# exosports/transit

Hardware: AMD Instinct MI355X
Metric: wavenumber-points*layers/sec (CH4 2-4um emission spectrum) (higher is better)
Workload: dtype f64; 1 GPU; BASELINE configs[1]: CH4-demo-shaped emission: 2500-5000 cm-1 @1 cm-1, wnosamp 2160, CH4 lines, eclipse, 5 angles, H2-H2 CIA; n_wn=2501, n_layers=100, layers_needed=81, n_lines=1000000, parallelism=one GPU

## Files before the change

transit_amd/csrc/hip/trx_api.hip:

```cpp
#include <hip/hip_runtime.h>
#include <rccl/rccl.h>
#include <dlfcn.h>

#include <algorithm>
#include <chrono>
#include <cmath>
#include <cstdio>
#include <cstdlib>
#include <cstring>
#include <atomic>
#include <condition_variable>
#include <memory>
#include <mutex>
#include <string>
#include <thread>
#include <vector>

#include "transit_hip.h"
#include "trx_kernels.hip.h"
#include "trx_walk.hip.h"
#include "trx_rows.hip.h"
#include "trx_tail.hip.h"
#include "trx_lanes.hip.h"
#include "trx_bands.hip.h"
// ... 15 lines not shown
  void release() { if (p) { (void)hipFree(p); p = nullptr; bytes = 0; } }
  template <class T> T *as() const { return (T *)p; }
};

struct PinnedBuf {
  void *p = nullptr, *dev = nullptr; size_t bytes = 0;
  ~PinnedBuf() { release(); }
  void release() { if (p) { (void)hipHostFree(p); p = dev = nullptr; bytes = 0; } }
};

struct DevView {
  void *p = nullptr;
  template <class T> T *as() const { return (T *)p; }
};

struct BandSet {
  int32_t nbands = 0; int64_t npieces = 0;
  DevBuf d_bands, d_pieces, d_w, d_part;
  PinnedBuf h_out;
};

struct PixelSet {
  int64_t npix = 0; double cut = 0;
  DevBuf d_centre, d_fwhm;
};
struct ObservedSet {
  int32_t nexp = 0, nseg = 0; int64_t npix = 0;
  DevBuf d_seg, d_data, d_weight, d_gain;
  std::vector<int64_t> seg;
};
struct FilterSet {
  int32_t ncomp = 0, npad = 0, nexp = 0, nseg = 0; int64_t npix = 0, ntiles = 0;
  DevBuf d_fwd, d_back, d_tiles;
};
struct PixelRun { const PixelSet *set; int32_t nshift; const ObservedSet *obs = nullptr; const FilterSet *filt = nullptr; };

struct Switches {
  bool no_row_copy = false;
  bool no_rows32 = false;
  bool row_staging = true;
  long long row_m8_from = 768;
  bool packed_walk = true; int packed_max_layers = 10;
  int xcd_map = 1;
  bool no_binrec = false;
  bool lanes_walk = true, lanes_force = false;
  int lanes_parts_most = 4;
  bool ray_tail = true;
  bool cia_sums = true;
  bool cia_segments = true;
  bool cia_window = true;
  bool two_queues = true;
  bool tail_direct = true;
  bool range_reach = true;
  bool shard_frames = true;
};

}

struct trx_handle {
  int device = 0;
  hipStream_t stream = nullptr, stream2 = nullptr;
  hipStream_t stream4 = nullptr;
  std::vector<hipEvent_t> ev_ac, ev_cb;
  hipEvent_t ev_walk1 = nullptr;
  hipEvent_t ev_inputs = nullptr, ev_cia = nullptr, ev_join = nullptr, ev_run_a = nullptr, ev_run_b = nullptr;
  std::string err;

  double wn_i = 0, wn_d = 0, odwn = 0; int64_t nwn = 0, nown = 0, lo = 0, hi = 0, nsh = 0; int osamp = 1;
  int niso = 0, nmol = 0;
  std::vector<double> iso_mass, iso_ratio, mol_mass, mol_radius, mol_pol;
  std::vector<double> pair_csd, pair_sqrt;
  std::vector<int32_t> iso_imol, mol_is_h2;
  std::vector<double> iso_wmin, iso_wmax;
  int ndop = 0, nlor = 0;
  std::vector<double> adop, alor;
  std::vector<int32_t> psizeT; bool psize_mono = false;
  std::vector<double> dopthr;
  std::vector<double> lorthr;
  std::vector<int> guess_dop, guess_lor, guess_a0, guess_a1;
  std::vector<long> guess_npre;
  std::vector<double> iso_sqrtm;
  std::vector<double> dens_over_m;
  std::vector<int32_t> psize; std::vector<long long> poff; int64_t tab_n = 0;
  DevBuf d_adop, d_dopthr, d_e2tab, d_psize, d_poff, d_tab, d_tabT, d_poffT, d_gimod, d_gidiv;
  float *tab = nullptr; const float *tabT = nullptr; const long long *poffT = nullptr;
  DevBuf d_tabW, d_walkprof; const float *tabW = nullptr; bool tabw_ok = false;
  DevBuf d_tabW32, d_wp32; const float *tabW32 = nullptr; unsigned slab32 = 0;
  std::vector<std::pair<double, double>> recip_ok;
  int max_gcount = 0; DevBuf d_linebase, d_rinfo;
  Switches sw;
  int64_t nlines = 0, ngroups = 0, nadd = 0, ninrange = 0;
  DevBuf d_lgroup, d_wavn, d_elow, d_gf, d_iso, d_inr, d_gfirst, d_gcount, d_giown, d_giso, d_gwavn, d_gblock, d_cntge, d_cntsub;
  int sub_f = 1;
  LinesDev L{};
  HostBuf<double> h_gwavn; std::vector<int32_t> h_gblock; HostBuf<int32_t> h_cntge, h_gfirst, h_gcount;
  void *comm = nullptr; int nranks = 1, rank = 0;
  bool windowed() const { return lo > 0 || hi < nwn; }
  DevBuf d_cand, d_candrec; int64_t ncand = -1;
  DevBuf d_kmax;
  int kmax_parity = 0, kmax_nr = 0; bool kmax_clean = false;
  DevBuf d_walk, d_wbase, d_part[2];
  std::vector<int32_t> h_wbase; int nwaves = 0, ngw = 0; bool walk_ok = false;
  bool walk_temp_ok = true;
  struct Plan { bool built = false; DevBuf blo, bhi, off, binw, binrec; int64_t records = 0; };
  Plan plan[4];
  struct Cia { int nspec; int mol[2]; std::vector<double> wn, temp, cs, zt, uw, ruw, rh, wf, wb; DevBuf d_wn, d_temp, d_cs, d_zt, d_uw, d_ruw, d_rh, d_wf, d_wb; };
  std::vector<Cia> cia;
  DevBuf d_cia_ws;
  DevBuf d_SG, d_idop8, d_sticky, d_part3;
  DevBuf d_in; PinnedBuf h_in;
  DevBuf d_pm_f64, d_pm_i32;
  DevBuf d_xf;
  DevBuf d_small; DevView d_flags, d_status, d_counters; PinnedBuf h_small;
  DevBuf d_e, d_ecs, d_er, d_tau, d_last, d_intens, d_spec, d_acc, d_geom;
  bool has_grid = false; long og_nmol = 0, og_ntemp = 0, og_nlayer = 0, og_nwave = 0;
  std::vector<double> og_temp; std::vector<int32_t> og_molidx; DevBuf d_og_o, d_og_layer, d_og_itemp, d_iso_mx, d_pm;
  trx_stats stats{};
  std::vector<double> run_f64, run_geom, run_ipv; std::vector<int32_t> run_i32;
  std::vector<int> run_frame; std::vector<unsigned char> run_wide;
  std::vector<PlanStep> run_plan;
  std::vector<double> run_og_layer; std::vector<int> run_og_itemp;
  int hint_layers = 0;
  DevBuf d_e_saved; std::vector<uint8_t> saved;
  PinnedBuf h_spec;
  PinnedBuf h_tailblk;
  std::unique_ptr<BandSet> bands;
  DevBuf d_cpart; PinnedBuf h_contrib;
  std::unique_ptr<PixelSet> pixels;
  DevBuf d_pixshift, d_pixout;
  std::unique_ptr<ObservedSet> observed;
  DevBuf d_mom;
  std::unique_ptr<FilterSet> filter;
  DevBuf d_pixval;
};

namespace {

struct LogSink { trx_log_fn fn = nullptr; void *user = nullptr; int max_level = 0; };
LogSink &log_sink() { static LogSink s; return s; }
void log_msg(int level, const std::string &msg)
{
  const LogSink s = log_sink();
// ... 44 lines not shown
int ensure_small(trx_handle *h, int nlay)
{
  const size_t bytes = 128 + 24 * (size_t)nlay;
  if (const int rc = ensure(h, h->d_small, bytes)) return rc;
  char *base = (char *)h->d_small.p;
  h->d_flags.p = base; h->d_status.p = base + 64; h->d_counters.p = base + 128;
  return ensure_pinned(h, h->h_small, bytes);
}

template <class T>
int upload_raw(trx_handle *h, DevBuf &b, const T *p, size_t n)
{
  int rc = ensure(h, b, n * sizeof(T));
  if (rc) return rc;
  if (n) HIPCHK(h, hipMemcpyAsync(b.p, p, n * sizeof(T), hipMemcpyHostToDevice, h->stream));
  return TRX_OK;
}

template <class T>
int upload(trx_handle *h, DevBuf &b, const std::vector<T> &v)
{
  int rc = ensure(h, b, v.size() * sizeof(T));
  if (rc) return rc;
  if (!v.empty()) HIPCHK(h, hipMemcpyAsync(b.p, v.data(), v.size() * sizeof(T), hipMemcpyHostToDevice, h->stream));
  return TRX_OK;
}

template <class T>
int upload(trx_handle *h, DevBuf &b, const HostBuf<T> &v) { return upload_raw(h, b, v.data(), v.size()); }

void read_switches(Switches &w)
{
  auto set = [](const char *name) { return std::getenv(name) != nullptr; };
  auto num = [](const char *name, long long otherwise) { const char *e = std::getenv(name); return e ? std::atoll(e) : otherwise; };
  auto clamped = [&](const char *name, int lo, int hi, int otherwise) { return (int)std::max<long long>(lo, std::min<long long>(hi, num(name, otherwise))); };
  w.no_row_copy = set("TRX_NO_ROW_COPY");
  w.no_rows32 = set("TRX_NO_ROWS32");
  w.row_staging = !set("TRX_NO_ROW_STAGING");
  w.row_m8_from = num("TRX_ROWS_M8_FROM", w.row_m8_from);
  w.packed_walk = !set("TRX_NO_PACKED_WALK");
  w.packed_max_layers = clamped("TRX_PACKED_MAX_LAYERS", 1, 32, w.packed_max_layers);
  w.xcd_map = (int)num("TRX_XCD_MAP", w.xcd_map);
  w.no_binrec = set("TRX_NO_BINREC");
  const long long lanes = num("TRX_LANES_WALK", 1);
  w.lanes_walk = lanes != 0; w.lanes_force = lanes == 2;
  w.lanes_parts_most = clamped("TRX_LANES_PARTS", 2, 4, w.lanes_parts_most);
  w.ray_tail = num("TRX_RAY_TAIL", 1) != 0;
  w.cia_sums = num("TRX_CIA_SUMS", 1) != 0;
  w.cia_segments = num("TRX_CIA_SEGMENTS", 1) != 0;
  w.cia_window = num("TRX_CIA_WINDOW", 1) != 0;
  w.two_queues = num("TRX_TWO_QUEUES", 1) != 0;
  w.tail_direct = num("TRX_TAIL_DIRECT", 1) != 0;
  w.range_reach = num("TRX_RANGE_REACH", 1) != 0;
  w.shard_frames = num("TRX_SHARD_FRAMES", 1) != 0;
}

struct TableBuild { TablePlan P; DevBuf d_jobs; };

template <class F>
void for_job_batches(const std::vector<ProfileJob> &jobs, F fn)
{
  for (size_t j0 = 0; j0 < jobs.size(); j0 += 32768) fn(j0, (int)std::min<size_t>(32768, jobs.size() - j0));
}

int plan_into_handle(trx_handle *h, const trx_static *s, TableBuild &B)
{
  const char *text = "";
  const TablePlanError pe = plan_table(*s, B.P, &text);
  if (pe != kTablePlanOk) return fail(h, pe == kTablePlanArg ? TRX_E_ARG : TRX_E_UNSUPPORTED, text);
  h->adop = B.P.adop; h->alor = B.P.alor; h->psize = B.P.psize; h->poff = B.P.poff; h->tab_n = B.P.tab_n;
  h->psizeT = std::move(B.P.psizeT); h->psize_mono = B.P.psize_mono;
  if (!index_steps(h->adop.data(), s->ndop, h->dopthr)) return fail(h, TRX_E_ARG, "Doppler-width grid is not strictly increasing");
  if (!index_steps(h->alor.data(), s->nlor, h->lorthr)) h->lorthr.clear();
  return TRX_OK;
}

int upload_table_inputs(trx_handle *h, const trx_static *s, TableBuild &B)
{
  int rc;
  double coef[64]; long double fact = 1.0L;
  for (int n = 0; n < 64; n++) { if (n > 0) fact *= (long double)n; coef[n] = (double)(1.0L / (fact * (long double)(2 * n + 1))); }
  HIPCHK(h, hipMemcpyToSymbolAsync(HIP_SYMBOL(c_voigt_coef), coef, sizeof(coef), 0, hipMemcpyHostToDevice, h->stream));
  if ((rc = upload(h, B.d_jobs, B.P.jobs))) return rc;
  const size_t tab_alloc = table_alloc_floats(h->tab_n, s->osamp);
  if ((rc = ensure(h, h->d_tab, sizeof(float) * tab_alloc))) return rc;
  HIPCHK(h, hipMemsetAsync(h->d_tab.p, 0, sizeof(float) * tab_alloc, h->stream));
  h->tab = h->d_tab.as<float>() + kTabPad;
  if ((rc = upload(h, h->d_psize, h->psize)) || (rc = upload(h, h->d_poff, h->poff)) || (rc = upload(h, h->d_adop, h->adop)) ||
      (rc = upload(h, h->d_dopthr, h->dopthr))) return rc;
  std::vector<double> e2(64);
  for (int j = 0; j < 64; j++) e2[j] = (double)exp2l((long double)j / 64.0L);
  return upload(h, h->d_e2tab, e2);
}

void table_kernels(trx_handle *h, const TableBuild &B)
{
  const int m_limit = 64;
  const std::vector<ProfileJob> &jobs = B.P.jobs;
  for_job_batches(jobs, [&](size_t j0, int nj) {
    int maxnv = 0; bool any_wave = false;
    for (int j = 0; j < nj; j++) { maxnv = std::max(maxnv, jobs[j0 + j].nv); any_wave |= (jobs[j0 + j].regime == 2 && jobs[j0 + j].m > m_limit); }
    const int gx = std::max(1, std::min(64, (maxnv + 255) / 256));
    hipLaunchKernelGGL(k_voigt_bins, dim3(gx, nj), dim3(256), 0, h->stream, B.d_jobs.as<ProfileJob>() + j0, h->tab, m_limit);
    if (any_wave)
      hipLaunchKernelGGL(k_voigt_bins_wave, dim3(std::max(1, std::min(256, maxnv)), nj), dim3(64), 0, h->stream,
                         B.d_jobs.as<ProfileJob>() + j0, h->tab, m_limit);
// ... 176 lines not shown
    for (int64_t g = g0; g < g1; g++) { Q.lgroup[(size_t)G.first[g]] = (int32_t)g; Q.gimod[g] = G.iown[g] % s->osamp; Q.gidiv[g] = G.iown[g] / s->osamp; }
  });
  Q.T.lap("cnt_sub, lgroup, gimod");
}

int walk_ranges(trx_handle *h, const trx_static *s, const LinePrep &Q)
{
  h->walk_ok = s->osamp < (1 << 21) && h->tab_n < ((int64_t)1 << 28) && !Q.LG.first.empty();
  if (!h->walk_ok) return TRX_OK;
  const int ngw = h->ngw = groups_per_range((int64_t)Q.LG.first.size());
  h->h_wbase.assign(s->niso + 1, 0);
  for (int b = 0; b < s->niso; b++) h->h_wbase[b + 1] = h->h_wbase[b] + (Q.gblock[b + 1] - Q.gblock[b] + ngw - 1) / ngw;
  h->nwaves = h->h_wbase[s->niso];
  return upload(h, h->d_wbase, h->h_wbase);
}

int upload_lines(trx_handle *h, LinePrep &Q)
{
  LineGroups &G = Q.LG;
  int rc;
  if ((rc = upload(h, h->d_wavn, Q.wavn)) || (rc = upload(h, h->d_inr, Q.inr)) || (rc = upload(h, h->d_lgroup, Q.lgroup)) ||
      (rc = upload(h, h->d_gfirst, G.first)) || (rc = upload(h, h->d_gcount, G.count)) || (rc = upload(h, h->d_giown, G.iown)) ||
      (rc = upload(h, h->d_giso, G.iso)) || (rc = upload(h, h->d_gwavn, G.wavn)) || (rc = upload(h, h->d_gimod, Q.gimod)) ||
      (rc = upload(h, h->d_gidiv, Q.gidiv)) || (rc = upload(h, h->d_gblock, Q.gblock)) || (rc = upload(h, h->d_cntge, Q.cntge)) ||
      (rc = upload(h, h->d_cntsub, Q.cntsub)))
    return rc;
  HIPCHK(h, hipStreamSynchronize(h->stream));
  Q.T.lap("uploads + sync");
  h->h_gwavn = std::move(G.wavn); h->h_gblock = Q.gblock; h->h_cntge = std::move(Q.cntge); h->h_gfirst = std::move(G.first); h->h_gcount = std::move(G.count);
  Q.T.lap("host copies");
  LinesDev &L = h->L;
  L.nlines = Q.n; L.wavn = h->d_wavn.as<double>(); L.elow = h->d_elow.as<double>(); L.gf = h->d_gf.as<double>();
  L.iso = h->d_iso.as<int16_t>(); L.inrange = h->d_inr.as<uint8_t>(); L.lgroup = h->d_lgroup.as<int32_t>();
  L.ngroups = h->ngroups; L.gfirst = h->d_gfirst.as<int32_t>(); L.gcount = h->d_gcount.as<int32_t>();
  L.giown = h->d_giown.as<int32_t>(); L.giso = h->d_giso.as<int16_t>(); L.gwavn = h->d_gwavn.as<double>();
  L.gblock = h->d_gblock.as<int32_t>(); L.cnt_ge = h->d_cntge.as<int32_t>();
  return TRX_OK;
}

int walk_records(trx_handle *h, const trx_static *s, const LinePrep &Q)
{
  const int64_t n = Q.n; const LinesDev &L = h->L;
  int rc;
  if ((rc = ensure(h, h->d_walk, sizeof(WalkLine) * ((size_t)n + 1))) || (rc = ensure(h, h->d_linebase, sizeof(double) * ((size_t)n + 1)))) return rc;
  HIPCHK(h, hipMemsetAsync(h->d_linebase.p, 0, sizeof(double) * ((size_t)n + 1), h->stream));
  h->max_gcount = parallel_minmax<int>((int64_t)h->h_gcount.size(), Q.nth, 0, 0, [&](int64_t g, bool &) { return (int)h->h_gcount[(size_t)g]; }).hi;
  hipLaunchKernelGGL(k_walk_records, dim3((unsigned)((n + 256) / 256)), dim3(256), 0, h->stream, (long long)n, L.wavn, L.elow, L.gf,
                     L.lgroup, L.giown, s->osamp, h->d_walk.as<WalkLine>());
  hipLaunchKernelGGL(k_walk_marks, dim3((unsigned)((h->nwaves + 63) / 64)), dim3(64), 0, h->stream, h->nwaves, h->ngw, s->niso,
                     h->d_wbase.as<int32_t>(), L.gblock, L.gfirst, L.gcount, h->d_walk.as<WalkLine>(), h->d_linebase.as<double>());
  if ((rc = ensure(h, h->d_rinfo, sizeof(RangeInfo) * (size_t)std::max(h->nwaves, 1)))) return rc;
  hipLaunchKernelGGL(k_range_info, dim3((unsigned)((h->nwaves + 255) / 256)), dim3(256), 0, h->stream, h->nwaves, h->ngw, s->niso,
                     h->d_wbase.as<int32_t>(), L.gblock, L.gfirst, L.gcount, h->d_walk.as<WalkLine>(), s->osamp, h->d_rinfo.as<RangeInfo>());
  return TRX_OK;
}

int line_candidates(trx_handle *h, const trx_static *s, const LinePrep &Q)
{
  const int64_t n = Q.n; const LinesDev &L = h->L;
  h->ncand = -1;
  if (!(h->ninrange > 4096 && s->niso > 0)) return TRX_OK;
  const MinMax<double> e = parallel_minmax<double>(n, Q.nth, HUGE_VAL, -HUGE_VAL, [&](int64_t i, bool &use) { use = Q.inr[i]; return s->elow[i]; });
  CandGeom Gm{};
  Gm.e_min = e.lo; Gm.e_scale = e.hi > e.lo ? kCandGrid / (e.hi - e.lo) : 0.0;
  Gm.w_min = Q.wn0;  Gm.w_scale = Q.own_last > Q.wn0 ? kCandGrid / (Q.own_last - Q.wn0) : 0.0;
  const int cap = (int)std::max<int64_t>(4096, n / 8);
  DevBuf d_M, d_n;
  const size_t mbytes = sizeof(unsigned long long) * (size_t)s->niso * kCandGrid * kCandGrid;
  int rc;
  if ((rc = ensure(h, d_M, mbytes)) || (rc = ensure(h, d_n, sizeof(int))) || (rc = ensure(h, h->d_cand, sizeof(int32_t) * (size_t)cap))) return rc;
  HIPCHK(h, hipMemsetAsync(d_M.p, 0, mbytes, h->stream));
  HIPCHK(h, hipMemsetAsync(d_n.p, 0, sizeof(int), h->stream));
  const unsigned nb = (unsigned)((n + 255) / 256);
  hipLaunchKernelGGL(k_cand_cellmax, dim3(nb), dim3(256), 0, h->stream, (long long)n, L.wavn, L.elow, L.gf, L.iso, L.inrange, Gm, d_M.as<unsigned long long>());
  hipLaunchKernelGGL(k_cand_prefix, dim3((unsigned)s->niso), dim3(kCandGrid), 0, h->stream, d_M.as<unsigned long long>());
  hipLaunchKernelGGL(k_cand_select, dim3(nb), dim3(256), 0, h->stream, (long long)n, L.wavn, L.elow, L.gf, L.iso, L.inrange, Gm,
                     d_M.as<unsigned long long>(), h->d_cand.as<int32_t>(), d_n.as<int>(), cap);
  int nc = 0;
  HIPCHK(h, hipMemcpyAsync(&nc, d_n.p, sizeof(int), hipMemcpyDeviceToHost, h->stream));
  HIPCHK(h, hipStreamSynchronize(h->stream));
  HIPCHK(h, hipGetLastError());
  if (!(nc > 0 && nc <= cap)) return TRX_OK;
  h->ncand = nc;
  if ((rc = ensure(h, h->d_candrec, sizeof(CandLine) * (size_t)nc))) return rc;
  hipLaunchKernelGGL(k_cand_pack, dim3((unsigned)((nc + 255) / 256)), dim3(256), 0, h->stream, nc, h->d_cand.as<int32_t>(),
                     L.wavn, L.elow, L.gf, L.iso, L.inrange, h->d_candrec.as<CandLine>());
  HIPCHK(h, hipStreamSynchronize(h->stream));
  return TRX_OK;
}

int prepare_lines(trx_handle *h, const trx_static *s)
{
  LinePrep Q;
  const int64_t n = Q.n = s->nlines;
  Q.nth = create_threads();
  Q.wn0 = s->wn_i; Q.odwn = s->wn_d / s->osamp; Q.own_last = Q.wn0 + (double)(s->nown - 1) * Q.odwn;
  if (n > 2000000000LL) return fail(h, TRX_E_UNSUPPORTED, "more than 2^31 lines per handle");
  int rc_raw = TRX_OK;
  std::thread raw_up([&]() {
    (void)hipSetDevice(h->device);
    if ((rc_raw = upload_raw(h, h->d_elow, s->elow, (size_t)n)) || (rc_raw = upload_raw(h, h->d_gf, s->gf, (size_t)n)) ||
        (rc_raw = upload_raw(h, h->d_iso, s->isoid, (size_t)n))) return;
  });
  struct Joiner { std::thread &t; ~Joiner() { if (t.joinable()) t.join(); } } raw_join{raw_up};
  int rc;
  if ((rc = line_wavenumbers(h, s, Q)) || (rc = check_line_order(h, s, Q)) || (rc = group_and_check(h, s, Q))) return rc;
// ... 435 lines not shown

template <int NB>
void launch_walk(const WalkArgs &A, bool prof, unsigned nwaves, hipStream_t st)
{
  const dim3 grid((nwaves + kWalkWaves - 1) / kWalkWaves), block(64 * kWalkWaves);
  if (prof) hipLaunchKernelGGL((k_line_walk<NB, true>), grid, block, 0, st, A);
  else if constexpr (NB >= 8) {
    if (A.nc <= 32) hipLaunchKernelGGL((k_line_walk<NB, false, 2>), grid, block, 0, st, A);
    else            hipLaunchKernelGGL((k_line_walk<NB, false>), grid, block, 0, st, A);
  }
  else      hipLaunchKernelGGL((k_line_walk<NB, false>), grid, block, 0, st, A);
}

struct PendingCombine {
  bool valid = false;
  CombineArgs C{}; hipStream_t sc = nullptr; hipEvent_t ev_walk = nullptr, ev_done = nullptr; bool cross = false;
};

int launch_combine(trx_handle *h, PendingCombine &pc, Spans *sp)
{
  if (!pc.valid) return TRX_OK;
  pc.valid = false;
  if (pc.cross) HIPCHK(h, hipStreamWaitEvent(pc.sc, pc.ev_walk, 0));
  if (sp && sp->begin(Spans::kAccum, pc.sc)) return fail(h, TRX_E_HIP, "event");
  hipLaunchKernelGGL(k_walk_combine, dim3((unsigned)((h->nsh + kCombineBins - 1) / kCombineBins)), dim3(64 * kCombineBins), 0, pc.sc, pc.C);
  if (sp && sp->end(pc.sc)) return fail(h, TRX_E_HIP, "event");
  if (pc.cross && pc.ev_done) HIPCHK(h, hipEventRecord(pc.ev_done, pc.sc));
  return TRX_OK;
}

int walk_chunk(trx_handle *h, const LayerDev &Y, const double *d_wcut, int nb, int r_top, int nc, const SweepMode &M, Spans *sp,
               int parity, hipStream_t st_comb, hipEvent_t ev_walk, hipEvent_t ev_reuse = nullptr, hipEvent_t ev_done = nullptr,
               PendingCombine *defer = nullptr ,
               int *form_out = nullptr )
{
  hipStream_t st = M.st ? M.st : h->stream;
  WalkPlan P{}; trx_handle::Plan *pl = nullptr;
  int rc = walk_plan(h, nb, st, P, pl);
  if (rc) return rc;
  DevBuf &part = h->d_part[parity & 1];
  if (!M.permol) { h->stats.walk_steps++; h->stats.walk_records += pl->records; h->stats.walk_record_lanes += pl->records * nc; }
  const size_t pbytes = sizeof(double) * kWalkLayers * (size_t)std::max<int64_t>(pl->records, 1);
  if (part.bytes < pbytes) {
    HIPCHK(h, hipStreamSynchronize(st));
    HIPCHK(h, hipStreamSynchronize(h->stream4));
    if ((rc = ensure(h, part, pbytes))) return rc;
  }
  if (ev_reuse) HIPCHK(h, hipStreamWaitEvent(st, ev_reuse, 0));
  WalkArgs A{};
  A.lines = h->d_walk.as<WalkLine>(); A.rinfo = h->d_rinfo.as<RangeInfo>(); A.gfirst = h->d_gfirst.as<int32_t>(); A.gcount = h->d_gcount.as<int32_t>();
  A.gblock = h->d_gblock.as<int32_t>(); A.P = P;
  A.niso = h->niso; A.nlor = h->nlor; A.ndop = h->ndop; A.osamp = h->osamp; A.lo = h->lo; A.hi = h->hi;
  A.wn_i = h->wn_i; A.odwn = h->odwn; A.range_reach = h->sw.range_reach && h->psize_mono;
  A.r_top = r_top; A.nc = nc; A.Y = Y; A.wcut = d_wcut; A.kmax = M.d_kmax; A.ethresh = M.ethresh;
  A.nmx = M.nmx; A.iso_mx = M.d_iso_mx; A.permol = M.permol; A.sticky_idop = M.d_sticky;
  A.dthr = h->d_dopthr.as<double>(); A.e2tab = h->d_e2tab.as<double>();
  A.psize = h->d_psize.as<int32_t>(); A.poff = h->d_poff.as<long long>();
  A.table = h->tab; A.zero_index = h->tab_n;
  A.tabw = h->tabW; A.walkprof = h->d_walkprof.as<WalkProfile>();
  A.tabw32 = h->tabW32; A.wp32 = h->tabW32 ? h->d_wp32.as<uint32_t>() : nullptr; A.slab32 = h->slab32;
  A.xcd_map = h->sw.xcd_map & 2;
  A.part = part.as<double>(); A.counters = M.prof ? h->d_counters.as<unsigned long long>() : nullptr;
  A.flags = h->d_flags.as<int>(); A.last = M.skip_done ? h->d_last.as<int>() : nullptr; A.eager = M.eager;
  unsigned nw = (unsigned)h->nwaves;
  A.nseg = 0;
  if (h->windowed() && h->niso <= kWalkSegs && nw > 0) {
    const int Rc = nb / 2 - 1;
    const long long klo = std::max<long long>(0, h->lo - Rc - 1), khi = std::min<long long>(h->nwn - 1, h->hi - 1 + Rc);
    int cum = 0, ns = 0;
    for (int b = 0; b < h->niso; b++) {
      const int gb0 = h->h_gblock[b], gb1 = h->h_gblock[b + 1];
      if (gb0 == gb1) continue;
      const int32_t *cg = &h->h_cntge[(size_t)b * (h->nwn + 1)];
      const int ga = cg[khi + 1], gz = h->lo - Rc - 1 <= 0 ? gb1 - gb0 : cg[klo];
      const int wa = h->h_wbase[b] + ga / h->ngw, wz = h->h_wbase[b] + (gz + h->ngw - 1) / h->ngw;
      if (wz <= wa) continue;
      A.seg_w0[ns] = wa; A.seg_cum[ns] = cum; cum += wz - wa; ns++;
    }
    A.seg_cum[ns] = cum; A.nseg = ns;
    nw = (unsigned)cum;
    if (ns == 0) { A.nseg = 1; A.seg_w0[0] = 0; A.seg_cum[0] = 0; A.seg_cum[1] = 0; }
  }
  const bool lanes_prod = nw > 0 && A.tabw != nullptr && nb >= 8 && nc <= kLanesMaxLayers && h->sw.lanes_walk &&
                          h->max_gcount <= kLanesMaxGroup && (h->ngroups >= 8 * h->nwn || h->sw.lanes_force);
  const bool packed_prod = !lanes_prod && nw > 0 && A.tabw != nullptr && nc <= h->sw.packed_max_layers && h->sw.packed_walk;
  const bool lanes = lanes_prod && !M.prof, packed = packed_prod && !M.prof;
  const int form_prod = lanes_prod ? 1 : packed_prod ? 2 : 0, form = lanes ? 1 : packed ? 2 : 0;
  if (form_out) *form_out = form_prod;
  if (!M.permol) { h->stats.walk_form_steps[form_prod]++; h->stats.walk_form_layers[form_prod] += nc; h->stats.walk_form_record_lanes[form_prod] += pl->records * nc; }
  if (sp && sp->begin(form == 1 ? Spans::kWalkLanes : form == 2 ? Spans::kWalkPacked : Spans::kWalk, st)) return fail(h, TRX_E_HIP, "event");
  if (lanes) {
    LanesExtra X{h->d_linebase.as<double>()};
    A.xcd_map = h->sw.xcd_map & 1;
    if (log_sink().fn && log_sink().max_level >= TRX_LOG_DEBUG)
      log_msg(TRX_LOG_DEBUG, "walk: lanes = lines, " + std::to_string(nc) + " layers, " + std::to_string(nb) + "-bin frames, " +
                             std::to_string(lanes_parts(nc, h->sw.lanes_parts_most)) + " lanes per layer");
    const dim3 grid((nw + kLanesWaves - 1) / kLanesWaves), block(64 * kLanesWaves);
    const size_t lds = lanes_lds_bytes(nc, h->ndop);
    const int parts = lanes_parts(nc, h->sw.lanes_parts_most);
    if (nb == 8) {
      if (parts == 4)      hipLaunchKernelGGL((k_line_walk_lanes<8, 5, 4>), grid, block, lds, st, A, X);
      else if (parts == 3) hipLaunchKernelGGL((k_line_walk_lanes<8, 5, 3>), grid, block, lds, st, A, X);
      else                 hipLaunchKernelGGL((k_line_walk_lanes<8, 5, 2>), grid, block, lds, st, A, X);
    } else {
      if (parts == 4)      hipLaunchKernelGGL((k_line_walk_lanes<16, 2, 4>), grid, block, lds, st, A, X);
      else if (parts == 3) hipLaunchKernelGGL((k_line_walk_lanes<16, 2, 3>), grid, block, lds, st, A, X);
// ... 1975 lines not shown
```

transit_amd/csrc/hip/trx_device.h:

```cpp
#pragma once
#include <stdint.h>

#include "../trx_numerics.h"

namespace trx {

constexpr int kMaxChunk   = 32;
constexpr int kMaxIso     = 256;
constexpr int kMaxAngles  = 16;
constexpr int kMaxDop     = 256;
constexpr int kTileBins   = 4;
constexpr int kTabPad     = 512;

struct ProfileJob {
  int64_t off;
  int32_t nv;
  int32_t regime;
  int32_t m;
  int32_t pad;
  double  half;
  double  sub;
  double  alphaL, alphaD;
  int64_t first_bin;
};
// ... 37 lines not shown
constexpr int kRowSpan = 256;
constexpr int kRowMaxT = 512;
constexpr int kRowTail = kRowMaxT + kRowSpan + 8;

TRX_HD void walk_row_layout(int K, int &front, int &stride)
{
  if (K <= 8) { front = 4; stride = 16; }
  else if (K <= 16) { front = 8; stride = 32; }
  else { front = 8; stride = (K + 16 + 15) & ~15; }
}

TRX_HD bool walk_may_stick(double wn_i, double odwn, int osamp, int cell1, double wcut)
{
  return wn_i + ((double)cell1 * (double)osamp - 1.0) * odwn < wcut;
}

TRX_HD int walk_lane_reach(int ps_first, int ps_sticky, bool may_stick)
{
  const int st = may_stick ? ps_sticky : 0;
  return ps_first > st ? ps_first : st;
}

TRX_HD int walk_range_reach(int psm_s, int lanes_max, bool use_range)
{
  return use_range && lanes_max < psm_s ? lanes_max : psm_s;
}

TRX_HD bool walk_group_out_of_reach(int imod, int osamp, int reach)
{
  return imod > reach && imod < osamp - reach;
}

TRX_HD unsigned walk_cand_slots(int NB, int imod, int osamp, int reach, int psq, int psr)
{
  if (NB == 2) return (imod <= reach ? 1u : 0u) | (osamp - imod <= reach ? 2u : 0u);
  const int Rc = NB / 2 - 1;
  const int klo = Rc - psq + (imod > psr ? 1 : 0), khi = Rc + psq + (imod + psr >= osamp ? 1 : 0);
  return ((2u << khi) - 1u) & ~((1u << klo) - 1u);
}

constexpr int32_t kRangeNoExit = 0;
TRX_HD int32_t walk_range_phases(bool one_cell, int osamp, int imod_min, int imod_max)
{
  if (!one_cell || osamp >= 65536) return kRangeNoExit;
  return (int32_t)((uint32_t)imod_min | ((uint32_t)imod_max << 16));
}

TRX_HD bool walk_range_out_of_reach(int32_t phases, int osamp, int reach)
{
  const int lo = (int)((uint32_t)phases & 0xffffu), hi = (int)((uint32_t)phases >> 16);
  return walk_group_out_of_reach(lo, osamp, reach) && walk_group_out_of_reach(hi, osamp, reach);
}

struct alignas(16) WalkProfile {
  uint32_t centre4;
  int32_t rowb;
  int32_t psr;
  int32_t ps;
};

}
```

transit_amd/csrc/hip/trx_walk.hip.h:

```cpp
#pragma once
#include "trx_kernels.hip.h"

namespace trx {

constexpr int    kCandGrid = 128;
constexpr double kCandEps  = 1e-9;

struct CandGeom { double e_min, e_scale, w_min, w_scale; };

__device__ __forceinline__ int cand_cell(double x, double x0, double scale)
{
  const double c = (x - x0) * scale;
  int k = (c > 0) ? (int)fmin(c, (double)(kCandGrid - 1)) : 0;
  return k;
}

__global__ __launch_bounds__(256)
void k_cand_cellmax(long long n, const double *__restrict__ wavn, const double *__restrict__ elow,
                    const double *__restrict__ gf, const int16_t *__restrict__ iso, const uint8_t *__restrict__ inr,
                    CandGeom Gm, unsigned long long *__restrict__ M )
{
  const long long i = (long long)blockIdx.x * 256 + threadIdx.x;
  if (i >= n || !inr[i]) return;
  const double g = gf[i];
// ... 249 lines not shown
    R.wavn = wavn[i]; R.elow = elow[i]; R.gf = gf[i];
    const int g = lgroup[i];
    if (g >= 0) { const int io = giown[g]; R.meta = 1 | ((io % osamp) << 3); R.cell = io / osamp; }
  }
  out[i] = R;
}

__global__ __launch_bounds__(64)
void k_walk_marks(int nwaves, int ngw, int niso, const int32_t *__restrict__ wbase, const int32_t *__restrict__ gblock,
                  const int32_t *__restrict__ gfirst, const int32_t *__restrict__ gcount, WalkLine *__restrict__ out,
                  double *__restrict__ linebase )
{
  const int w = blockIdx.x * 64 + threadIdx.x;
  if (w >= nwaves) return;
  int b = 0;
  while (b + 1 < niso && w >= wbase[b + 1]) b++;
  const int g0 = gblock[b] + (w - wbase[b]) * ngw, g1 = min(g0 + ngw, gblock[b + 1]);
  for (int g = g0; g < g1; g++) {
    const int la = gfirst[g], lz = la + gcount[g] - 1;
    out[lz].meta |= 2;
    for (int l = la + 1; l <= lz; l++) out[l].cell = out[la].cell;
  }
  const int l0 = gfirst[g0], l1 = gfirst[g1 - 1] + gcount[g1 - 1];
  double w0 = HUGE_VAL;
  for (int l = l0; l < l1; l++) {
    const double wv = out[l].wavn;
    if (l == l0 || w0 - wv > kRebaseSpan) { out[l].meta |= 4; w0 = wv; }
    linebase[l] = w0;
  }
}

struct alignas(32) RangeInfo { int32_t l0, l1, b, cell0; double wavn0; int32_t cell1, phases; };

__global__ __launch_bounds__(256)
void k_range_info(int nwaves, int ngw, int niso, const int32_t *__restrict__ wbase, const int32_t *__restrict__ gblock,
                  const int32_t *__restrict__ gfirst, const int32_t *__restrict__ gcount, const WalkLine *__restrict__ lines,
                  int osamp, RangeInfo *__restrict__ out)
{
  const int w = blockIdx.x * 256 + threadIdx.x;
  if (w >= nwaves) return;
  int b = 0;
  while (b + 1 < niso && w >= wbase[b + 1]) b++;
  const int g0 = gblock[b] + (w - wbase[b]) * ngw, g1 = min(g0 + ngw, gblock[b + 1]);
  RangeInfo R{};
  R.l0 = gfirst[g0]; R.l1 = gfirst[g1 - 1] + gcount[g1 - 1]; R.b = b;
  R.cell0 = lines[R.l0].cell; R.wavn0 = lines[R.l0].wavn; R.cell1 = lines[gfirst[g1 - 1]].cell;
  int imin = osamp, imax = 0;
  if (R.cell0 == R.cell1)
    for (int g = g0; g < g1; g++) { const int im = lines[gfirst[g]].meta >> 3; imin = min(imin, im); imax = max(imax, im); }
  R.phases = walk_range_phases(R.cell0 == R.cell1, osamp, imin, imax);
  out[w] = R;
}

__device__ __forceinline__ int xcd_block(int i, int n)
{
  const int x = i & 7, k = i >> 3, q = n >> 3, r = n & 7;
  return x * q + min(x, r) + k;
}

struct WalkArgs {
  const WalkLine *lines;
  const RangeInfo *rinfo;
  const int32_t *gfirst, *gcount, *gblock;
  WalkPlan P;
  int niso, nlor, ndop, osamp;
  double wn_i, odwn;
  int range_reach;
  long long lo, hi;
  int r_top, nc;
  LayerDev Y; const double *wcut;
  const double *kmax;
  double ethresh;
  int nmx; const int32_t *iso_mx; int permol;
  const int *sticky_idop;
  const double *dthr;
  const double *e2tab;
  const int32_t *psize; const long long *poff;
  long long zero_index;
  const float *table;
  const float *tabw; const WalkProfile *walkprof;
  int xcd_map;
  const float *tabw32; const uint32_t *wp32;
  unsigned slab32;
  double *part;
  unsigned long long *counters;
  const int *flags; const int *last; int eager;
  int nseg; int seg_w0[kWalkSegs]; int seg_cum[kWalkSegs + 1];
};

__device__ __forceinline__ double exp_small(double x, double c24)
{
  double p = __builtin_fma(0x1.1111111111111p-7, x, c24);
  p = __builtin_fma(p, x, 0x1.5555555555555p-3);
  p = __builtin_fma(p, x, 0.5);
  p = __builtin_fma(p, x, 1.0);
  p = __builtin_fma(p, x, 1.0);
  return p;
}
__device__ __forceinline__ double exp_small(double x)
{
  double p = 0x1.1111111111111p-7;
  p = __builtin_fma(p, x, 0x1.5555555555555p-5);
  p = __builtin_fma(p, x, 0x1.5555555555555p-3);
  p = __builtin_fma(p, x, 0.5);
  p = __builtin_fma(p, x, 1.0);
  p = __builtin_fma(p, x, 1.0);
  return p;
}

constexpr int kWalkWaves = 4;

template <int NB, bool PROF, int LPL = 1>
__global__ __launch_bounds__(64 * kWalkWaves)
void k_line_walk(WalkArgs A)
{
  constexpr int Rc = NB / 2 - 1;
  constexpr int NS = NB / LPL;
  constexpr bool ROWS = !PROF && NB >= kWalkRowsFrom;
  static_assert(LPL == 1 || (LPL == 2 && ROWS && NS >= 4), "lane pairs: row form, frames of 8+ bins");
  if (!A.eager && A.flags[0] == 0) return;
  const int wv = __builtin_amdgcn_readfirstlane(threadIdx.x >> 6);
  int w = (A.xcd_map ? xcd_block(blockIdx.x, gridDim.x) : (int)blockIdx.x) * kWalkWaves + wv;
  if (A.nseg > 0) {
    if (w >= A.seg_cum[A.nseg]) return;
    int sgm = 0;
    while (sgm + 1 < A.nseg && w >= A.seg_cum[sgm + 1]) sgm++;
    w = A.seg_w0[sgm] + (w - A.seg_cum[sgm]);
  }
  if (w >= A.P.nwaves) return;
  const int lane = threadIdx.x & 63;
  const int blo = A.P.blo[w], bhi = A.P.bhi[w];
  if (bhi < blo) return;
  if (A.last) {
    bool open = false;
    for (int j = blo + lane; j <= bhi; j += 64) open |= A.last[j - A.lo] < 0;
    if (__ballot(open) == 0ull) return;
  }
  __shared__ double s_thr_w[kWalkWaves][kMaxDop + 1];
  __shared__ double s_e2_w[kWalkWaves][64];
  double *s_thr = s_thr_w[wv], *s_e2 = s_e2_w[wv];
  for (int i = lane; i <= A.ndop; i += 64) s_thr[i] = A.dthr[i];
  s_e2[lane] = A.e2tab[lane];
  __builtin_amdgcn_wave_barrier();

  const RangeInfo RI = A.rinfo[w];
  const int b = __builtin_amdgcn_readfirstlane(RI.b), l0 = __builtin_amdgcn_readfirstlane(RI.l0), l1 = __builtin_amdgcn_readfirstlane(RI.l1);
  const long long rec0 = A.P.off[w];

  const int li = LPL == 1 ? lane : (lane >> 1), part = LPL == 1 ? 0 : (lane & 1);
  const bool valid = li < A.nc;
  const int r = A.r_top - (valid ? li : 0), ri = r * A.niso + b;
  const int psm_l = valid ? A.Y.psmax[ri] : 0;
  const int mx = A.nmx == 1 ? 0 : A.iso_mx[b];
  const double ct = valid ? A.Y.negc_over_t[r] : 0.0;
  const double f = A.Y.strength_f[ri], dens = A.permol ? 1.0 : A.Y.density[ri];
  const double lim = A.ethresh * A.kmax[(long long)r * A.nmx + mx];
  const double wc = A.wcut[ri], ad = A.Y.alphad[ri];
  const int il = A.Y.ilor[ri];
  const int idst = A.sticky_idop[ri];
  const int idop0 = A.Y.idop0[ri];

  auto fill_zero = [&](int ja, int jb) {
    ja = max(ja, blo); jb = min(jb, bhi);
    if (valid && part == 0) for (int j = ja; j <= jb; j++) A.part[(rec0 + (j - blo)) * kWalkLayers + li] = 0.0;
  };

  const int psm_s = __builtin_amdgcn_readfirstlane(wave_max_i(psm_l));
  const bool range_reach = !PROF && A.range_reach != 0;
  const int phases = __builtin_amdgcn_readfirstlane(RI.phases), cell1 = __builtin_amdgcn_readfirstlane(RI.cell1);
  if (range_reach && walk_range_out_of_reach(phases, A.osamp, psm_s)) { fill_zero(blo, bhi); return; }

  const int ps_st = A.psize[idst * A.nlor + il];
  const unsigned vo_st = (unsigned)(A.poff[idst * A.nlor + il] + ps_st);
  const int lo32 = (int)A.lo, hi32 = (int)A.hi;
  const bool interior = cell1 - Rc >= lo32 && __builtin_amdgcn_readfirstlane(RI.cell0) + Rc + 1 < hi32;

  int lo_i = index_from(s_thr, ad * RI.wavn0, idop0);
  double thr_lo = s_thr[lo_i];
  int ps_cur = A.psize[lo_i * A.nlor + il];
  unsigned vo_cur = 4u * (unsigned)(A.poff[lo_i * A.nlor + il] + ps_cur);
  const unsigned vo_st8 = 4u * vo_st;
  WalkProfile wp_cur{}, wp_st{};
  if (ROWS) { wp_cur = A.walkprof[lo_i * A.nlor + il]; wp_st = A.walkprof[idst * A.nlor + il]; }

  const int reach_l = valid ? walk_lane_reach(ps_cur, ps_st, walk_may_stick(A.wn_i, A.odwn, A.osamp, cell1, wc)) : 0;
  const int psm = walk_range_reach(psm_s, range_reach ? __builtin_amdgcn_readfirstlane(wave_max_i(reach_l)) : psm_s, range_reach);
  if (range_reach && walk_range_out_of_reach(phases, A.osamp, psm)) { fill_zero(blo, bhi); return; }
  const int psq = psm / A.osamp, psr = psm - psq * A.osamp;

  double acc[NS];
#pragma unroll
  for (int k = 0; k < NS; k++) acc[k] = 0.0;
  int jc = __builtin_amdgcn_readfirstlane(RI.cell0);
  unsigned long long nb = 0, nev = 0, nsk = 0;

  auto flush = [&](int k, double v, bool mine = true) {
    const int j = jc - Rc + part * NS + k;
    if (valid && mine && j >= blo && j <= bhi) A.part[(rec0 + (j - blo)) * kWalkLayers + li] = v;
  };

  double pk = 0.0;
  double c24 = 0x1.5555555555555p-5;
  asm volatile("" : "+v"(c24));
  int cell = jc, imod = 0;
  unsigned cand = 0u;
  float pv_p[NS]; double kk_p = 0.0;
#pragma unroll
  for (int k = 0; k < NS; k++) pv_p[k] = 0.f;
  auto settle = [&]() {
#pragma unroll
    for (int k = 0; k < NS; k++) acc[k] = __builtin_fma(kk_p, (double)pv_p[k], acc[k]);
  };
  const char *tab_k[NB];
#pragma unroll
  for (int k = 0; k < NB; k++) tab_k[k] = (const char *)A.table + 4LL * (k - Rc - 1) * A.osamp;
  const unsigned vzero = 4u * (unsigned)(A.zero_index + (long long)(Rc + 1) * A.osamp);
  const unsigned cell8 = 4u * (unsigned)A.osamp;
  const char *tabw_base = (const char *)A.tabw - 4 * (Rc + 1);

  typedef const __attribute__((address_space(4))) double *ScalarF64;
  typedef const __attribute__((address_space(4))) int32_t *ScalarI32;
  ScalarF64 rp = (ScalarF64)(A.lines + l0);
  double L_wavn = rp[0], L_elow = rp[1], L_gf = rp[2];
  int L_meta = ((ScalarI32)rp)[6] | 4, L_cell = ((ScalarI32)rp)[7];
  double c0 = 0.0, E0 = 1.0, wav_a = L_wavn;
  for (int left = l1 - l0; left > 0; left--) {
    rp += 4;
    const double N_wavn = rp[0], N_elow = rp[1], N_gf = rp[2];
    const int N_meta = ((ScalarI32)rp)[6], N_cell = ((ScalarI32)rp)[7];
    if (L_meta & 4) {
      const double t0 = ct * L_wavn;
      E0 = exp_neg(t0, s_e2, c24); c0 = -t0;
    }
    if (L_meta & 1) {
      cell = L_cell; imod = L_meta >> 3; wav_a = L_wavn;
      cand = walk_cand_slots(NB, imod, A.osamp, psm, psq, psr);
      if (!interior) {
#pragma unroll
        for (int k = 0; k < NB; k++) { const int j = cell - Rc + k; if (j < lo32 || j >= hi32) cand &= ~(1u << k); }
      }
      if (PROF) cand |= 0x80000000u;
    }
    if (cand) {
      const double e1 = exp_neg(ct * L_elow, s_e2, c24);
      const double q = __builtin_fma(-E0, exp_small(__builtin_fma(ct, L_wavn, c0), c24), 1.0);
      pk += L_gf * e1 * q;
      if (L_meta & 2) {
        const double pkf = pk * f;
        pk = 0.0;
        const bool below = pkf < lim;
        if (PROF && cell >= lo32 && cell < hi32 && valid) { if (below) nsk++; else nev++; }
        const double kk = pkf * dens;
        const double v = ad * wav_a;
        if (__any(v < thr_lo)) {
          do {
            if (v < thr_lo) {
              lo_i--; thr_lo = s_thr[lo_i];
              ps_cur = A.psize[lo_i * A.nlor + il];
              vo_cur = 4u * (unsigned)(A.poff[lo_i * A.nlor + il] + ps_cur);
              if (ROWS) wp_cur = A.walkprof[lo_i * A.nlor + il];
            }
          } while (__any(v < thr_lo));
        }
        const bool own = wav_a >= wc;
        const int ps = own ? ps_cur : ps_st;
        const unsigned vo8 = own ? vo_cur : vo_st8;
        const bool act = valid && !below;
        settle();
        if (cell != jc) {
          int sh = jc - cell;
          if (sh >= NB) {
#pragma unroll
            for (int k = 0; k < NS; k++) { flush(k, acc[k]); acc[k] = 0.0; }
            fill_zero(cell + Rc + 2, jc - Rc - 1);
            jc = cell;
          } else {
            for (; sh > 0; sh--) {
              flush(NS - 1, acc[NS - 1], part == LPL - 1);
              double carry = 0.0;
// ... 270 lines not shown
```

Baseline: 886.0 million wavenumber-points*layers/s.

## Trim walk line ranges to groups within profile reach using per-wave group table

```diff
diff --git a/transit_amd/csrc/hip/trx_api.hip b/transit_amd/csrc/hip/trx_api.hip
--- a/transit_amd/csrc/hip/trx_api.hip
+++ b/transit_amd/csrc/hip/trx_api.hip
@@ -91,6 +91,7 @@
   bool two_queues = true;
   bool tail_direct = true;
   bool range_reach = true;
+  bool range_trim = true;
   bool shard_frames = true;
 };
 
@@ -127,6 +128,7 @@
   DevBuf d_tabW32, d_wp32; const float *tabW32 = nullptr; unsigned slab32 = 0;
   std::vector<std::pair<double, double>> recip_ok;
   int max_gcount = 0; DevBuf d_linebase, d_rinfo;
+  DevBuf d_gtab;
   Switches sw;
   int64_t nlines = 0, ngroups = 0, nadd = 0, ninrange = 0;
   DevBuf d_lgroup, d_wavn, d_elow, d_gf, d_iso, d_inr, d_gfirst, d_gcount, d_giown, d_giso, d_gwavn, d_gblock, d_cntge, d_cntsub;
@@ -277,6 +279,7 @@
   w.two_queues = num("TRX_TWO_QUEUES", 1) != 0;
   w.tail_direct = num("TRX_TAIL_DIRECT", 1) != 0;
   w.range_reach = num("TRX_RANGE_REACH", 1) != 0;
+  w.range_trim = num("TRX_RANGE_TRIM", 1) != 0;
   w.shard_frames = num("TRX_SHARD_FRAMES", 1) != 0;
 }
 
@@ -559,6 +562,10 @@
   if ((rc = ensure(h, h->d_rinfo, sizeof(RangeInfo) * (size_t)std::max(h->nwaves, 1)))) return rc;
   hipLaunchKernelGGL(k_range_info, dim3((unsigned)((h->nwaves + 255) / 256)), dim3(256), 0, h->stream, h->nwaves, h->ngw, s->niso,
                      h->d_wbase.as<int32_t>(), L.gblock, L.gfirst, L.gcount, h->d_walk.as<WalkLine>(), s->osamp, h->d_rinfo.as<RangeInfo>());
+  const size_t nslots = (size_t)std::max(h->nwaves, 1) * kTrimSlots;
+  if ((rc = ensure(h, h->d_gtab, sizeof(uint32_t) * nslots))) return rc;
+  hipLaunchKernelGGL(k_range_groups, dim3((unsigned)((nslots + 255) / 256)), dim3(256), 0, h->stream, h->nwaves, h->ngw, s->niso,
+                     h->d_wbase.as<int32_t>(), L.gblock, L.gfirst, h->d_walk.as<WalkLine>(), s->osamp, h->d_gtab.as<uint32_t>());
   return TRX_OK;
 }
 
@@ -1100,6 +1107,7 @@
   A.gblock = h->d_gblock.as<int32_t>(); A.P = P;
   A.niso = h->niso; A.nlor = h->nlor; A.ndop = h->ndop; A.osamp = h->osamp; A.lo = h->lo; A.hi = h->hi;
   A.wn_i = h->wn_i; A.odwn = h->odwn; A.range_reach = h->sw.range_reach && h->psize_mono;
+  A.gtab = h->sw.range_trim ? h->d_gtab.as<uint32_t>() : nullptr; A.linebase = h->d_linebase.as<double>();
   A.r_top = r_top; A.nc = nc; A.Y = Y; A.wcut = d_wcut; A.kmax = M.d_kmax; A.ethresh = M.ethresh;
   A.nmx = M.nmx; A.iso_mx = M.d_iso_mx; A.permol = M.permol; A.sticky_idop = M.d_sticky;
   A.dthr = h->d_dopthr.as<double>(); A.e2tab = h->d_e2tab.as<double>();
diff --git a/transit_amd/csrc/hip/trx_device.h b/transit_amd/csrc/hip/trx_device.h
--- a/transit_amd/csrc/hip/trx_device.h
+++ b/transit_amd/csrc/hip/trx_device.h
@@ -113,6 +113,29 @@
   return walk_group_out_of_reach(lo, osamp, reach) && walk_group_out_of_reach(hi, osamp, reach);
 }
 
+constexpr int kTrimSlots = 64;
+constexpr uint32_t kTrimPad = 0xffffffffu;
+
+TRX_HD bool walk_trim_encodable(int osamp, int ngw, int last_anchor_offset)
+{
+  return osamp < 65536 && ngw <= kTrimSlots && last_anchor_offset < 65536;
+}
+TRX_HD uint32_t walk_trim_word(int phase, int anchor_offset) { return (uint32_t)phase | ((uint32_t)anchor_offset << 16); }
+TRX_HD int walk_trim_phase(uint32_t word) { return (int)(word & 0xffffu); }
+TRX_HD int walk_trim_offset(uint32_t word) { return (int)(word >> 16); }
+TRX_HD bool walk_trim_is_pad(uint32_t word) { return (word & 0xffffu) == 0xffffu; }
+
+TRX_HD bool walk_trim_live(uint32_t word, int osamp, int reach)
+{
+  return !walk_trim_is_pad(word) && !walk_group_out_of_reach(walk_trim_phase(word), osamp, reach);
+}
+
+TRX_HD int walk_trim_begin(int l0, uint32_t word_first) { return l0 + walk_trim_offset(word_first); }
+TRX_HD int walk_trim_end(int l0, int l1, int last_live, uint32_t word_behind)
+{
+  return last_live + 1 < kTrimSlots && !walk_trim_is_pad(word_behind) ? l0 + walk_trim_offset(word_behind) : l1;
+}
+
 struct alignas(16) WalkProfile {
   uint32_t centre4;
   int32_t rowb;
diff --git a/transit_amd/csrc/hip/trx_walk.hip.h b/transit_amd/csrc/hip/trx_walk.hip.h
--- a/transit_amd/csrc/hip/trx_walk.hip.h
+++ b/transit_amd/csrc/hip/trx_walk.hip.h
@@ -325,6 +325,25 @@
   out[w] = R;
 }
 
+__global__ __launch_bounds__(256)
+void k_range_groups(int nwaves, int ngw, int niso, const int32_t *__restrict__ wbase, const int32_t *__restrict__ gblock,
+                    const int32_t *__restrict__ gfirst, const WalkLine *__restrict__ lines, int osamp, uint32_t *__restrict__ out )
+{
+  const long long t = (long long)blockIdx.x * 256 + threadIdx.x;
+  if (t >= (long long)nwaves * kTrimSlots) return;
+  const int w = (int)(t / kTrimSlots), slot = (int)(t % kTrimSlots);
+  int b = 0;
+  while (b + 1 < niso && w >= wbase[b + 1]) b++;
+  const int g0 = gblock[b] + (w - wbase[b]) * ngw, g1 = min(g0 + ngw, gblock[b + 1]);
+  const int l0 = gfirst[g0];
+  uint32_t word = kTrimPad;
+  if (walk_trim_encodable(osamp, ngw, gfirst[g1 - 1] - l0) && slot < g1 - g0) {
+    const int la = gfirst[g0 + slot];
+    word = walk_trim_word(lines[la].meta >> 3, la - l0);
+  }
+  out[t] = word;
+}
+
 __device__ __forceinline__ int xcd_block(int i, int n)
 {
   const int x = i & 7, k = i >> 3, q = n >> 3, r = n & 7;
@@ -339,6 +358,8 @@
   int niso, nlor, ndop, osamp;
   double wn_i, odwn;
   int range_reach;
+  const uint32_t *gtab;
+  const double *linebase;
   long long lo, hi;
   int r_top, nc;
   LayerDev Y; const double *wcut;
@@ -404,6 +425,10 @@
   const int lane = threadIdx.x & 63;
   const int blo = A.P.blo[w], bhi = A.P.bhi[w];
   if (bhi < blo) return;
+  const bool range_reach = !PROF && A.range_reach != 0;
+  const bool range_trim = range_reach && A.gtab != nullptr;
+  uint32_t gword = kTrimPad;
+  if (range_trim) gword = A.gtab[(long long)w * kTrimSlots + lane];
   if (A.last) {
     bool open = false;
     for (int j = blo + lane; j <= bhi; j += 64) open |= A.last[j - A.lo] < 0;
@@ -412,9 +437,6 @@
   __shared__ double s_thr_w[kWalkWaves][kMaxDop + 1];
   __shared__ double s_e2_w[kWalkWaves][64];
   double *s_thr = s_thr_w[wv], *s_e2 = s_e2_w[wv];
-  for (int i = lane; i <= A.ndop; i += 64) s_thr[i] = A.dthr[i];
-  s_e2[lane] = A.e2tab[lane];
-  __builtin_amdgcn_wave_barrier();
 
   const RangeInfo RI = A.rinfo[w];
   const int b = __builtin_amdgcn_readfirstlane(RI.b), l0 = __builtin_amdgcn_readfirstlane(RI.l0), l1 = __builtin_amdgcn_readfirstlane(RI.l1);
@@ -439,9 +461,12 @@
   };
 
   const int psm_s = __builtin_amdgcn_readfirstlane(wave_max_i(psm_l));
-  const bool range_reach = !PROF && A.range_reach != 0;
   const int phases = __builtin_amdgcn_readfirstlane(RI.phases), cell1 = __builtin_amdgcn_readfirstlane(RI.cell1);
   if (range_reach && walk_range_out_of_reach(phases, A.osamp, psm_s)) { fill_zero(blo, bhi); return; }
+
+  for (int i = lane; i <= A.ndop; i += 64) s_thr[i] = A.dthr[i];
+  s_e2[lane] = A.e2tab[lane];
+  __builtin_amdgcn_wave_barrier();
 
   const int ps_st = A.psize[idst * A.nlor + il];
   const unsigned vo_st = (unsigned)(A.poff[idst * A.nlor + il] + ps_st);
@@ -458,7 +483,17 @@
 
   const int reach_l = valid ? walk_lane_reach(ps_cur, ps_st, walk_may_stick(A.wn_i, A.odwn, A.osamp, cell1, wc)) : 0;
   const int psm = walk_range_reach(psm_s, range_reach ? __builtin_amdgcn_readfirstlane(wave_max_i(reach_l)) : psm_s, range_reach);
-  if (range_reach && walk_range_out_of_reach(phases, A.osamp, psm)) { fill_zero(blo, bhi); return; }
+  int l_a = l0, l_z = l1;
+  bool trimmed = false;
+  if (range_trim && (uint32_t)__builtin_amdgcn_readfirstlane((int)gword) != kTrimPad) {
+    const unsigned long long live = __ballot(walk_trim_live(gword, A.osamp, psm));
+    if (live == 0ull) { fill_zero(blo, bhi); return; }
+    const int first = __builtin_ctzll(live), last = 63 - __builtin_clzll(live);
+    l_a = walk_trim_begin(l0, (uint32_t)__builtin_amdgcn_readlane((int)gword, first));
+    l_z = walk_trim_end(l0, l1, last, (uint32_t)__builtin_amdgcn_readlane((int)gword, (last + 1) & 63));
+    trimmed = true;
+  }
+  else if (range_reach && walk_range_out_of_reach(phases, A.osamp, psm)) { fill_zero(blo, bhi); return; }
   const int psq = psm / A.osamp, psr = psm - psq * A.osamp;
 
   double acc[NS];
@@ -493,11 +528,16 @@
 
   typedef const __attribute__((address_space(4))) double *ScalarF64;
   typedef const __attribute__((address_space(4))) int32_t *ScalarI32;
-  ScalarF64 rp = (ScalarF64)(A.lines + l0);
+  ScalarF64 rp = (ScalarF64)(A.lines + l_a);
   double L_wavn = rp[0], L_elow = rp[1], L_gf = rp[2];
-  int L_meta = ((ScalarI32)rp)[6] | 4, L_cell = ((ScalarI32)rp)[7];
+  int L_meta = ((ScalarI32)rp)[6], L_cell = ((ScalarI32)rp)[7];
   double c0 = 0.0, E0 = 1.0, wav_a = L_wavn;
-  for (int left = l1 - l0; left > 0; left--) {
+  if (trimmed) {
+    const double t0 = ct * ((ScalarF64)A.linebase)[l_a];
+    E0 = exp_neg(t0, s_e2, c24); c0 = -t0;
+  }
+  else L_meta |= 4;
+  for (int left = l_z - l_a; left > 0; left--) {
     rp += 4;
     const double N_wavn = rp[0], N_elow = rp[1], N_gf = rp[2];
     const int N_meta = ((ScalarI32)rp)[6], N_cell = ((ScalarI32)rp)[7];
```

Measured after the change: 896.2 million wavenumber-points*layers/s (median of 6 runs). No clear change (+1.2%).
